# VincentStimper/normalizing-flows

Hardware: AMD Instinct MI355X
Metric: samples/sec + NLL (nats/dim), 32-layer RQ-NSF d=64 B=65536 (higher is better)
Workload: dtype f32; 1 GPU; BASELINE configs[1]: log_prob of 32 x [CoupledRQS(d=64, 2 blocks, 128 hidden, K=8, tail 3) + LULinearPermute(64)] + DiagGaussian, batch 65536 rows/GPU, N(0,I) inputs, sigma=0.01 perturbed seeded weights; rows_per_gpu=65536, global_rows=65536, layers=32, launch=hipGraph replay, parallelism=dp1

## Files before the change

include/nf_mi355x.h:

```cpp
#ifndef NF_MI355X_H
#define NF_MI355X_H

#include <stdint.h>

#ifdef __cplusplus
extern "C" {
#endif

typedef void *nf_stream_t;

enum { NF_OK = 0, NF_EIO = -5, NF_EFAULT = -14, NF_EINVAL = -22, NF_ERANGE = -34, NF_ENOTSUP = -95 };
enum { NF_F32 = 0, NF_F64 = 1 };
enum { NF_LD_WRITE = 0, NF_LD_ADD = 1, NF_LD_SUB = -1 };
enum { NF_TAILS_NONE = 0, NF_TAILS_LINEAR = 1, NF_TAILS_CIRCULAR = 2, NF_TAILS_FEATURE = 3  };
enum { NF_SCALE_EXP = 0, NF_SCALE_SIGMOID = 1, NF_SCALE_SIGMOID_INV = 2, NF_SCALE_NONE = 3 };
enum { NF_RQS_DENSITY = 0, NF_RQS_SAMPLE_IDENTITY = 1, NF_RQS_SAMPLE_TRANSFORM = 2 };

const char *nf_version(void);
const char *nf_strerror(int code);
int nf_mfma_clock_probe(void *out2_u64, void *sink_f32, int iters, nf_stream_t stream);
int nf_max_bins(void);
int nf_persistent_workgroups(void);

int nf_rqs_spline(const void *x, const void *w, int64_t ldw, const void *h, int64_t ldh, const void *d,
// ... 41 lines not shown
                                void *grad_ud, int dtype, const int32_t *tails_t, const void *bound_t,
                                const int32_t *tails_i, const void *bound_i, nf_stream_t stream);

int nf_rqs_fused_final_row(int K, int g, int rb, int rho);
#define NF_RQS_COMPACT_DIFF (1 << 16)
int nf_rqs_fused_compact_row(int K, int rb, int rho);
int64_t nf_rqs_fused_pack_size(int nI, int nT, int hidden, int num_blocks, int K);
int nf_rqs_fused_pack(void *wpack, const void *w_init, const void *b_init, const void *const *w_blocks,
                      const void *const *b_blocks, const void *w_final, const void *b_final, const void *uw,
                      const void *uh, const void *ud, int nI, int nT, int hidden, int num_blocks, int K,
                      double tail_bound, double min_bin_width, double min_bin_height, double min_derivative,
                      nf_stream_t stream);
int nf_rqs_fused_pack_lu(void *wpack, int num_blocks, const int64_t *perm, const void *lower_entries,
                         const void *upper_entries, const void *unconstrained_upper_diag, const void *bias, int D,
                         double eps, int K, nf_stream_t stream);
int nf_rqs_fused(const void *x, void *y, void *logdet, const void *wpack, int mask_parity, int fuse_lu, int64_t B,
                 int D, int hidden, int num_blocks, int K, double tail_bound, double min_bin_width,
                 double min_bin_height, double min_derivative, int direction, int acc, nf_stream_t stream);
int nf_rqs_fused_chain(const void *x, void *y, void *logdet, const void *const *wpacks, const int *mask_parities,
                       int num_layers, int fuse_lu, int64_t B, int D, int hidden, int num_blocks, int K,
                       double tail_bound, double min_bin_width, double min_bin_height, double min_derivative,
                       int direction, int acc, nf_stream_t stream);
int nf_rqs_fused_small_batch(int enable);

int nf_rqs_fused_pack_final(void *wpack, const void *w_final, const void *b_final, const void *uw, const void *uh,
                            const void *ud, int hidden, int num_blocks, int K, double tail_bound, double min_bin_width,
                            double min_bin_height, double min_derivative, nf_stream_t stream);
int nf_rqs_fused_train_fwd(const void *x, const void *h2, void *y, void *logdet, void *cond_out, const void *wpack,
                           int mask_parity, int64_t B, int D, int hidden, int num_blocks, int K, double tail_bound,
                           double min_bin_width, double min_bin_height, double min_derivative, int acc, nf_stream_t stream);
int nf_rqs_fused_pack_all(void *wpack, const void *w_init, const void *b_init, const void *const *w_blocks,
                          const void *const *b_blocks, const void *w_final, const void *b_final, const void *uw, const void *uh,
                          const void *ud, int hidden, int num_blocks, int K, double tail_bound, double min_bin_width,
                          double min_bin_height, double min_derivative, void *wfull, void *wpad, const void *identity_idx,
                          nf_stream_t stream);
int nf_rqs_fused_train_full_fwd(const void *x, void *y, void *logdet, void *cond_out, void *act_out, const void *wpack,
                                int mask_parity, int64_t B, int D, int hidden, int num_blocks, int K, double tail_bound,
                                double min_bin_width, double min_bin_height, double min_derivative, int acc, nf_stream_t stream);
int nf_rqs_fused_pack_all_multi(const void *table, int n_layers, int hidden, int num_blocks, int K, double tail_bound,
                                double min_bin_width, double min_bin_height, double min_derivative, nf_stream_t stream);
int nf_rqs_coupling_bwd_p24(const void *x, const void *grad_y, const void *grad_logdet, const void *cond24, const void *uw,
                            const void *uh, const void *ud, const int64_t *identity_idx, int nI, const int64_t *transform_idx,
                            int nT, int64_t B, int D, double tail_bound, double min_bin_width, double min_bin_height,
                            double min_derivative, double wh_div, void *grad_x, void *grad_cond24, void *grad_uw,
                            void *grad_uh, void *grad_ud, nf_stream_t stream);

// ... 322 lines not shown
```

normalizing-flows_amd/config.py:

```python
fused_gemm = "f32"


def set_fused_gemm(mode):
    global fused_gemm
    if mode not in ("f32", "bf16x3"):
        raise ValueError("fused_gemm must be 'f32' or 'bf16x3'")
    fused_gemm = mode


glow_level_chains = True


def set_glow_level_chains(mode=True):
    global glow_level_chains
    glow_level_chains = bool(mode)


def set_roctx(mode=True):
    from . import _prof
    _prof.enabled = bool(mode)


wgrad_pair = True

# ... 111 lines not shown
    global train_prepack
    train_prepack = bool(mode)


maf_halves = True


def set_maf_halves(mode=True):
    global maf_halves
    maf_halves = bool(mode)


maf_tri = True


def set_maf_tri(mode=True):
    global maf_tri
    maf_tri = bool(mode)


def set_fused_chain(mode=True):
    global fused_chain
    fused_chain = bool(mode)


lu_matvec2 = True


def set_lu_matvec2(mode=True):
    global lu_matvec2
    lu_matvec2 = bool(mode)


made_fused = True


def set_made_fused(mode=True):
    global made_fused
    made_fused = bool(mode)


made_train = True


def set_made_train(mode=True):
    global made_train
# ... 175 lines not shown
```

normalizing-flows_amd/core.py:

```python
import torch
from . import _keys
from . import config as _config
from torch import nn

from . import _prepack
from .flows.base import run_flow
from .flows.mixing import LULinearPermute
from .flows.neural_spline import CoupledRationalQuadraticSpline


def invalidate_caches(module):
    for m in module.modules():
        for k in list(m.__dict__.keys()):
            if k.endswith("_cache") and not k.startswith("__"):
                v = m.__dict__[k]
                m.__dict__[k] = {} if isinstance(v, dict) else None
        if hasattr(m, "refresh_graphs"):
            m.refresh_graphs()
    _realnvp_cache.clear()


def _pair_signature(crqs):
    p = crqs.prqct
    return (p.features, p.transform_net.hidden_features, len(p.transform_net.blocks), p.num_bins, p.tail_bound,
# ... 323 lines not shown
        for o in obj:
            _cached_tensors(o, out, depth + 1)
    elif isinstance(obj, dict) and depth < 4:
        for o in obj.values():
            _cached_tensors(o, out, depth + 1)


def _packed_blobs(owner):
    out = []
    if owner is not None:
        for m in owner.modules():
            for k, v in m.__dict__.items():
                if k.endswith("_cache"):
                    _cached_tensors(v, out)
    _cached_tensors(list(_realnvp_cache.values()), out)
    return out


class _GraphCache:

    def __init__(self, owner=None):
        self.enabled = False
        self.graphs = {}
        self.stamp, self.sig = _keys.stamp(), None
        self.owner = None if owner is None else __import__("weakref").ref(owner)

    def clear(self):
        self.graphs = {}

    def run(self, key, fn, *inputs):
        if not self.enabled:
            return fn(*inputs)
        if self.sig is None or self.stamp != _keys.stamp():
            owner = self.owner() if self.owner is not None else None
            sig = _keys.signature(owner.parameters()) if owner is not None else _keys.stamp()
            if self.sig is not None and sig != self.sig:
                self.graphs = {}
            self.sig, self.stamp = sig, _keys.stamp()
        entry = self.graphs.get(key)
        if entry is None:
            static_in = [t.clone() for t in inputs]
            _config._graph_recording += 1
            try:
                s = torch.cuda.Stream()
                s.wait_stream(torch.cuda.current_stream())
                with torch.cuda.stream(s):
                    fn(*static_in)
                torch.cuda.current_stream().wait_stream(s)
                g = torch.cuda.CUDAGraph()
                with torch.cuda.graph(g):
                    static_out = fn(*static_in)
            finally:
                _config._graph_recording -= 1
            entry = (g, static_in, static_out, _packed_blobs(self.owner() if self.owner is not None else None))
            self.graphs[key] = entry
        g, static_in, static_out = entry[:3]
        for dst, src in zip(static_in, inputs):
            dst.copy_(src)
        g.replay()
        if torch.is_tensor(static_out):
            return static_out.clone()
# ... 43 lines not shown
    def inverse(self, x):
        for i in range(len(self.flows) - 1, -1, -1):
            x, _ = self.flows[i].inverse(x)
        return x

    def inverse_and_log_det(self, x):
        log_det = torch.zeros(len(x), dtype=x.dtype, device=x.device)
        x = run_chain(self.flows, x, True, log_det, +1)
        return x, log_det

    def _train_pad_rows(self, x):
        B = x.shape[0] if x.dim() == 2 else 0
        if (B < 1024 or B % 64 == 0 or not _config.train_pad_batch or not x.is_cuda or x.dtype != torch.float32 or x.shape[1] != 64
                or not torch.is_grad_enabled() or not (_config.train_pair and _config.train_bwd_onecall)):
            return 0
        fl = list(self.flows)
        for a, b in zip(fl[:-1], fl[1:]):
            if (isinstance(a, CoupledRationalQuadraticSpline) and isinstance(b, LULinearPermute) and b.linear.features == 64
                    and a.prqct._train_full_ok(x, None, False) and all(p.requires_grad for p in a.parameters())
                    and all(p.requires_grad for p in b.parameters())):
                return (-B) % 64 if all(_row_wise(f) for f in fl) else 0
        return 0

    def _log_prob_impl(self, x):
        pad = self._train_pad_rows(x)
        if pad:
            B = x.shape[0]
            x = torch.cat([x, x.new_zeros((pad, x.shape[1]))])
        log_q = torch.zeros(len(x), dtype=x.dtype, device=x.device)
        z = run_chain(self.flows, x, True, log_q, +1)
        if hasattr(self.q0, "_log_prob_acc"):
            self.q0._log_prob_acc(z, log_q, +1)
        else:
            log_q += self.q0.log_prob(z)
        return log_q[:B] if pad else log_q

    def log_prob(self, x):
        if self._graphs.enabled and torch.is_grad_enabled() and any(p.requires_grad for p in self.parameters()):
            return self._log_prob_impl(x)
        return self._graphs.run(("log_prob", tuple(x.shape), x.dtype), self._log_prob_impl, x)

    def forward_kld(self, x):
        return -torch.mean(self.log_prob(x))

    def _sample_impl(self, eps):
        z, log_q = self.q0.from_noise(eps)
        z = run_chain(self.flows, z, False, log_q, -1)
        return z, log_q

    def sample_from_noise(self, eps):
        if self._graphs.enabled and torch.is_grad_enabled() and any(p.requires_grad for p in self.parameters()):
            return self._sample_impl(eps)
        return self._graphs.run(("sample", tuple(eps.shape), eps.dtype), self._sample_impl, eps)

    def sample(self, num_samples=1):
        if hasattr(self.q0, "from_noise"):
            eps = torch.randn((num_samples,) + tuple(self.q0.shape), dtype=self.q0.loc.dtype,
                              device=self.q0.loc.device)
            return self.sample_from_noise(eps)
        z, log_q = self.q0(num_samples)
        for flow in self.flows:
            z = run_flow(flow, z, False, log_q, -1)
# ... 319 lines not shown
```

normalizing-flows_amd/csrc/affine.hip:

```cpp
#include "common.hpp"

namespace nf {

template <typename T>
__global__ void __launch_bounds__(256)
masked_affine_kernel(const T *__restrict__ z, const T *__restrict__ b, const T *__restrict__ s,
                     const T *__restrict__ t, T *__restrict__ y, T *__restrict__ logdet, int64_t B, int64_t inner,
                     int direction, int acc) {
    __shared__ T sred[16];
    if constexpr (sizeof(T) == 4) {
        if (inner <= 256 && (inner & 3) == 0) {
            typedef float v4 __attribute__((ext_vector_type(4)));
            const int L4 = (int)inner >> 2;
            int P = 1;
            while (P < L4) P <<= 1;
            const int rpw = 64 / P, lane = threadIdx.x & 63, rin = lane / P, i = lane - rin * P;
            const int64_t wave = ((int64_t)blockIdx.x * blockDim.x + threadIdx.x) >> 6;
            const int64_t nwaves = ((int64_t)gridDim.x * blockDim.x) >> 6;
            const bool col_on = i < L4;
            v4 bi = {0.0f, 0.0f, 0.0f, 0.0f};
            if (col_on) bi = *reinterpret_cast<const v4 *>(reinterpret_cast<const float *>(b) + 4 * i);
            for (int64_t r0 = wave * rpw; r0 < B; r0 += nwaves * rpw) {
                const int64_t r = r0 + rin;
                const bool on = r < B && col_on;
// ... 213 lines not shown
                    for (int e = 0; e < 4; ++e) {
                        const float q = (zv[e] - mu[e]) * inv[e];
                        a += 0.5f * q * q;
                    }
                }
                for (int off = P >> 1; off >= 1; off >>= 1) a += __shfl_xor(a, off, 64);
                if (r < B && i == 0) ld_store(reinterpret_cast<float *>(out) + r, (float)cst - a, acc);
            }
            return;
        }
    }
    for (int64_t r = wave; r < B; r += nwaves) {
        T a = T(0);
        for (int64_t j = lane; j < d; j += 64) {
            const T ls = log_scale[j] + ls_shift;
            const T q = (z[r * d + j] - loc[j]) / M<T>::exp(ls);
            a += ls + T(0.5) * q * q;
        }
        a = wave_sum(a);
        if (lane == 0) ld_store(out + r, cst - a, acc);
    }
}

template <typename T>
__global__ void __launch_bounds__(256)
squeeze_kernel(const T *__restrict__ z, T *__restrict__ y, int64_t B, int C, int H, int W, int direction) {
    const int64_t N = B * (int64_t)C * H * W;
    for (int64_t i = (int64_t)blockIdx.x * blockDim.x + threadIdx.x; i < N; i += (int64_t)gridDim.x * blockDim.x) {
        if (direction == 0) {
            const int Co = C / 4, Ho = 2 * H, Wo = 2 * W;
            int64_t r = i;
            const int wo = (int)(r % Wo); r /= Wo;
            const int ho = (int)(r % Ho); r /= Ho;
            const int co = (int)(r % Co); r /= Co;
            const int ci = 4 * co + 2 * (ho & 1) + (wo & 1);
            y[i] = z[((r * C + ci) * H + (ho >> 1)) * W + (wo >> 1)];
        } else {
            const int Co = 4 * C, Ho = H / 2, Wo = W / 2;
            int64_t r = i;
            const int wo = (int)(r % Wo); r /= Wo;
            const int ho = (int)(r % Ho); r /= Ho;
            const int co = (int)(r % Co); r /= Co;
            const int ci = co >> 2, di = (co >> 1) & 1, dj = co & 1;
            y[i] = z[((r * C + ci) * H + (2 * ho + di)) * W + (2 * wo + dj)];
        }
    }
// ... 127 lines not shown
}

extern "C" int nf_diag_gaussian_log_prob(const void *z, const void *loc, const void *log_scale, double log_scale_shift,
                                         void *out, int64_t B, int64_t d, int acc, int dtype, nf_stream_t stream) {
    if (B < 0 || d < 1 || acc < NF_LD_SUB || acc > NF_LD_ADD) return NF_EINVAL;
    if (B == 0) return NF_OK;
    if (!z || !loc || !log_scale || !out) return NF_EFAULT;
    if (dtype == NF_F32 && d <= 256 && (d & 3) == 0 && nf_misaligned16(z, loc, log_scale)) return NF_EINVAL;
    hipStream_t st = (hipStream_t)stream;
    const double cst = -0.5 * (double)d * log(2.0 * M_PI);
    int grid = grid_for(B, 4);
    if (dtype == NF_F32 && d <= 256 && (d & 3) == 0) grid = grid_for(B * d / 4, 256);
    NF_DISPATCH(dtype,
                hipLaunchKernelGGL(diag_gaussian_kernel<float>, dim3(grid), dim3(256), 0, st, (const float *)z,
                                   (const float *)loc, (const float *)log_scale, (float)log_scale_shift, (float *)out,
                                   B, d, (float)cst, acc),
                hipLaunchKernelGGL(diag_gaussian_kernel<double>, dim3(grid), dim3(256), 0, st, (const double *)z,
                                   (const double *)loc, (const double *)log_scale, log_scale_shift, (double *)out, B,
                                   d, cst, acc));
    NF_CHECK_LAUNCH();
    return NF_OK;
}

extern "C" int nf_squeeze(const void *z, void *y, int64_t B, int C, int H, int W, int direction, int dtype,
                          nf_stream_t stream) {
    if (B < 0 || C < 1 || H < 1 || W < 1 || (direction != 0 && direction != 1)) return NF_EINVAL;
    if (direction == 0 && (C % 4)) return NF_EINVAL;
    if (direction == 1 && ((H % 2) || (W % 2))) return NF_EINVAL;
    if (B == 0) return NF_OK;
    if (!z || !y) return NF_EFAULT;
    hipStream_t st = (hipStream_t)stream;
    const int grid = grid_for(B * (int64_t)C * H * W, 256 * 4);
    NF_DISPATCH(dtype,
                hipLaunchKernelGGL(squeeze_kernel<float>, dim3(grid), dim3(256), 0, st, (const float *)z, (float *)y, B,
                                   C, H, W, direction),
                hipLaunchKernelGGL(squeeze_kernel<double>, dim3(grid), dim3(256), 0, st, (const double *)z,
                                   (double *)y, B, C, H, W, direction));
    NF_CHECK_LAUNCH();
    return NF_OK;
}

extern "C" int nf_maf_affine(const void *x, const void *params, void *y, void *logdet, int64_t B, int D, int direction,
                             int acc, int dtype, nf_stream_t stream) {
    if (B < 0 || D < 1 || (direction != 0 && direction != 1) || acc < NF_LD_SUB || acc > NF_LD_ADD) return NF_EINVAL;
    if (B == 0) return NF_OK;
    if (!x || !params || !y) return NF_EFAULT;
// ... 11 lines not shown
```

normalizing-flows_amd/csrc/common.hpp:

```cpp
#pragma once
#include <hip/hip_runtime.h>
#include <stdint.h>
#include <math.h>

#include "../../include/nf_mi355x.h"

#define NF_MAX_BINS 64
#define NF_WAVE 64

#ifdef NF_SAFE_WAITS
#define NF_WAIT_VMCNT(N) asm volatile("s_waitcnt vmcnt(0)" ::: "memory")
#else
#define NF_WAIT_VMCNT(N) asm volatile("s_waitcnt vmcnt(%0)" ::"n"(N) : "memory")
#endif

#define NF_DMA16(BASE, BYTE_OFF, LDS_DST)                                                                                          \
    do {                                                                                                                           \
        uint32_t m0__;                                                                                                             \
        const uint32_t ldsa__ = __builtin_amdgcn_readfirstlane((uint32_t)(uintptr_t)(LDS_DST));                                    \
        const uint64_t b64__ = (uint64_t)(uintptr_t)(BASE);                                                                        \
        const uint64_t sb__ = ((uint64_t)(uint32_t)__builtin_amdgcn_readfirstlane((uint32_t)(b64__ >> 32)) << 32) |                \
                              (uint32_t)__builtin_amdgcn_readfirstlane((uint32_t)b64__);                                           \
        asm volatile("s_mov_b32 %0, m0\n\ts_mov_b32 m0, %1\n\ts_nop 0\n\tglobal_load_lds_dwordx4 %2, %3\n\ts_mov_b32 m0, %0"      \
                     : "=&s"(m0__) : "s"(ldsa__), "v"((uint32_t)(BYTE_OFF)), "s"(sb__) : "memory");                                \
// ... 288 lines not shown
template <typename T> __device__ __forceinline__ T wave_sum(T v) {
#pragma unroll
    for (int o = 32; o > 0; o >>= 1) v += __shfl_xor(v, o, 64);
    return v;
}

template <typename T> __device__ __forceinline__ T block_sum(T v, T *scratch ) {
    v = wave_sum(v);
    const int lane = threadIdx.x & 63, wid = threadIdx.x >> 6, nw = (blockDim.x + 63) >> 6;
    __syncthreads();
    if (lane == 0) scratch[wid] = v;
    __syncthreads();
    T r = T(0);
    for (int i = 0; i < nw; ++i) r += scratch[i];
    return r;
}

template <typename T> __device__ __forceinline__ void ld_store(T *dst, T v, int acc) {
    if (acc == NF_LD_WRITE) *dst = v;
    else if (acc == NF_LD_ADD) *dst += v;
    else *dst -= v;
}

static inline int grid_for(int64_t work_items, int per_block, int max_blocks = 256 * 8) {
    int64_t g = (work_items + per_block - 1) / per_block;
    if (g < 1) g = 1;
    if (g > max_blocks) g = max_blocks;
    return (int)g;
}

constexpr int NF_PERSISTENT_WORKGROUPS = 256;
static inline int persistent_grid(int64_t ntiles) {
    return (int)(ntiles < NF_PERSISTENT_WORKGROUPS ? ntiles : NF_PERSISTENT_WORKGROUPS);
}

constexpr int NF_MAX_DEVICES = 64;
struct LdsOptIn {
    size_t opted[NF_MAX_DEVICES];
};
inline int opt_in_lds(const void *kernel, size_t lds, LdsOptIn &state) {
    if (lds <= 64 * 1024) return NF_OK;
    int dev = 0;
    if (hipGetDevice(&dev) != hipSuccess || dev < 0 || dev >= NF_MAX_DEVICES) return NF_EIO;
    if (lds <= state.opted[dev]) return NF_OK;
    if (hipFuncSetAttribute(kernel, hipFuncAttributeMaxDynamicSharedMemorySize, (int)lds) != hipSuccess) return NF_ENOTSUP;
    state.opted[dev] = lds;
// ... 5 lines not shown
```

normalizing-flows_amd/csrc/rqs_fused.hip:

```cpp
#include "fused_common.hpp"
#include <type_traits>

#define NF_TRAIN_STORE(ptr, val) __builtin_nontemporal_store((val), (ptr))

#ifdef NF_FUSED_SECONDARY
#define rqs_fused_kernel rqs_fused_kernel_nw4
#endif

namespace nf {

#ifndef NF_FUSED_SECONDARY
__global__ void pack_init_kernel(const float *__restrict__ W , const float *__restrict__ b, float *__restrict__ stage,
                                 float *__restrict__ bias_dst) {
    for (int i = blockIdx.x * blockDim.x + threadIdx.x; i < F_STAGE; i += gridDim.x * blockDim.x) {
        const int r4 = i & 3, lane = (i >> 2) & 63, s = (i >> 8) & 3, m = i >> 10;
        const int row = 32 * m + (lane & 31);
        const int k = 8 * s + 4 * (lane >> 5) + r4;
        stage[i] = W[row * F_NI + k];
    }
    for (int i = blockIdx.x * blockDim.x + threadIdx.x; i < 128; i += gridDim.x * blockDim.x) {
        const int reg = i & 15, hh = (i >> 4) & 1, m = i >> 5;
        bias_dst[i] = b[32 * m + 8 * (reg >> 2) + 4 * hh + (reg & 3)];
    }
}
// ... 288 lines not shown
    }
}

#ifndef NF_FUSED_WAVES
#define NF_FUSED_WAVES 8
#endif
constexpr int F_NW = NF_FUSED_WAVES;
constexpr int F_DMA_WAVES = 4 < F_NW ? 4 : F_NW;
constexpr int F_THREADS = 64 * F_NW;
constexpr int F_ROWS = 32 * F_NW;

struct FlowArgs {
    const float *blob[F_MAX_LAYERS];
    unsigned long long parity;
    int nlayers;
    int ngroups;
};

template <int DIR, bool LU, int TRAIN = 0, int KB = F_K, int HB = 4>
__global__ void __launch_bounds__(F_THREADS, 2)
rqs_fused_kernel(const float *__restrict__ x, float *__restrict__ y, float *__restrict__ logdet, FlowArgs fa,
                 int64_t B, int nblk, RqsParams<float> p, int acc, const float *__restrict__ h_in = nullptr,
                 float *__restrict__ cond_out = nullptr, float unscale = 1.0f, float *__restrict__ act_out = nullptr,
                 float *__restrict__ xlu_out = nullptr) {
    extern __shared__ __attribute__((aligned(16))) float smem[];
    constexpr int LA = (HB == 4 && !(DIR == 0 && LU) && TRAIN == 0) ? 1 : 2;
    static_assert(KB == 4 || KB == 8 || KB == 16, "bins");
    static_assert(!TRAIN || (KB == F_K && DIR == 0 && (!LU || TRAIN == 2)),
                  "the training variants: 8 bins, density direction; the fused LU only with the whole-layer forward (TRAIN = 2)");
    static_assert(HB == 4 || ((HB == 2 || HB == 1) && !TRAIN), "hidden row-blocks");
    constexpr bool COMPACT = KB == 8 && TRAIN == 0;
    constexpr bool RAW_RELU = !(KB == 16 && DIR == 0 && LU && HB == 4);
    auto relu_acc = [](float v) __attribute__((always_inline)) { return RAW_RELU ? relu_raw(v) : fmaxf(v, 0.0f); };
    constexpr bool PAIR_TAB = TRAIN == 0;
    constexpr int MP = 3 * KB, FPL = 16 / KB, GQ = KB / 4, TABW = 3 * (KB + 1);
    FusedLayout lay;
    lay.nblk = nblk;
    lay.K = KB;
    float *ring = smem;
    float *stash = ring + 2 * F_STAGE;
    float *small2 = stash + F_NW * 32 * 64;
    const int small_pitch = TRAIN ? lay.small_padded_legacy() : lay.small_padded();
    const int tid = threadIdx.x, lane = tid & 63, hh = lane >> 5;
    const int wid = __builtin_amdgcn_readfirstlane(tid >> 6);
    const int64_t row = (int64_t)blockIdx.x * F_ROWS + wid * 32 + (lane & 31);
    const bool valid = row < B;
    const int nhid = 2 * nblk * HB;
// ... 413 lines not shown
#pragma unroll
            for (int f = 0; f < FPL; ++f) element(g, f);
        }
        if (DIR == 0) uncond_group(g);
    }

    if (LU && DIR == 1) {
        float yin[32];
#pragma unroll
        for (int c = 0; c < 32; ++c) yin[c] = st[c * 64];
        const float *bsrc = small + lay.off_bias_lu(1) + hh * 16;
        f32x16 o0 = load_bias16(bsrc), o1 = load_bias16(bsrc + 32);
        lu_mm(acquire(), lane, yin, o0, o1);
#pragma unroll
        for (int c = 0; c < 16; ++c) {
            st[c * 64] = o0[c];
            st[(16 + c) * 64] = o1[c];
        }
        if (hh == 0) ld -= lu_lad;
    }
    }

    ld += __shfl_xor(ld, 32, 64);
    if (valid) {
#pragma unroll
        for (int Q = 0; Q < 4; ++Q) {
            f32x4 a, b;
#pragma unroll
            for (int c = 0; c < 4; ++c) {
                a[c] = st[(8 * Q + c) * 64];
                b[c] = st[(8 * Q + 4 + c) * 64];
            }
            float *dst = y + row * F_D + 16 * Q + 8 * hh;
            *reinterpret_cast<f32x4 *>(dst) = a;
            *reinterpret_cast<f32x4 *>(dst + 4) = b;
        }
        if (hh == 0) ld_store(logdet + row, ld, acc);
    }
}

#ifndef NF_FUSED_SECONDARY
struct PackAllArgs {
    const float *w_init, *b_init, *w_final, *b_final, *uw, *uh, *ud;
    const float *w_blk[32], *b_blk[32];
    int nblk;
    float *wfull, *wpad;
    const int64_t *iidx;
};
__device__ __forceinline__ void pack_all_body(const PackAllArgs &a, float *__restrict__ blob, float wh_scale,
                                              const RqsParams<float> &p) {
    FusedLayout lay;
    lay.nblk = a.nblk;
    float *small = blob + F_HDR, *stages = blob + lay.off_stages();
    const int nlin = 2 * a.nblk, nst = 1 + 4 * nlin + 24;
    const int64_t tid0 = (int64_t)blockIdx.x * blockDim.x + threadIdx.x, nth = (int64_t)gridDim.x * blockDim.x;
    for (int64_t i = tid0; i < (int64_t)nst * F_STAGE; i += nth) {
        const int st = (int)(i >> 12), j = (int)(i & (F_STAGE - 1));
        const int r4 = j & 3, lane = (j >> 2) & 63;
// ... 321 lines not shown
    if (!wpack || !perm || !lower_entries || !upper_entries || !unconstrained_upper_diag || !bias) return NF_EFAULT;
    hipStream_t st = (hipStream_t)stream;
    FusedLayout lay;
    lay.nblk = num_blocks;
    lay.K = K;
    float *blob = (float *)wpack;
    float *small = blob + F_HDR;
    float *stages = blob + lay.off_stages();
    const size_t lds = (size_t)4 * F_D * F_D * sizeof(double) + F_D * sizeof(int) + F_D * sizeof(double) + 64;
    static LdsOptIn opted = {};
    if (opt_in_lds(reinterpret_cast<const void *>(&pack_lu_kernel), lds, opted) != NF_OK) return NF_ENOTSUP;
    hipLaunchKernelGGL(pack_lu_kernel, dim3(1), dim3(256), lds, st, perm, (const float *)lower_entries,
                       (const float *)upper_entries, (const float *)unconstrained_upper_diag, (const float *)bias,
                       (float)eps, stages + (size_t)lay.lu_stage(0) * F_STAGE, stages + (size_t)lay.lu_stage(1) * F_STAGE,
                       small + lay.off_bias_lu(0), small + lay.off_bias_lu(1), blob);
    NF_CHECK_LAUNCH();
    return NF_OK;
}

#endif

template <int DIR, bool LU, int KB, int HB>
static int launch_fused(const void *x, void *y, void *logdet, const FlowArgs &fa, int64_t B, int num_blocks,
                        const RqsParams<float> &p, int acc, size_t lds, hipStream_t st) {
    static LdsOptIn opted = {};
    if (opt_in_lds(reinterpret_cast<const void *>(&rqs_fused_kernel<DIR, LU, false, KB, HB>), lds, opted) != NF_OK) return NF_ENOTSUP;
    const int grid = (int)((B + F_ROWS - 1) / F_ROWS);
    hipLaunchKernelGGL((rqs_fused_kernel<DIR, LU, false, KB, HB>), dim3(grid), dim3(F_THREADS), lds, st, (const float *)x, (float *)y,
                       (float *)logdet, fa, B, num_blocks, p, acc, (const float *)nullptr, (float *)nullptr, 1.0f);
    NF_CHECK_LAUNCH();
    return NF_OK;
}

static int chain_dispatch(const void *x, void *y, void *logdet, const FlowArgs &fa, int64_t B, int hidden, int num_blocks, int K,
                          const RqsParams<float> &p, int direction, int fuse_lu, int acc, hipStream_t st) {
    FusedLayout lay;
    lay.nblk = num_blocks;
    lay.K = K;
    const size_t lds = (size_t)(2 * F_STAGE + F_NW * 32 * 64 + 2 * lay.small_padded()) * sizeof(float);
    if (lds > 160 * 1024) return NF_ENOTSUP;
#define NF_FUSED_DISPATCH(KB, HB)                                                                                     \
    do {                                                                                                              \
        if (direction == 0)                                                                                           \
            return fuse_lu ? launch_fused<0, true, KB, HB>(x, y, logdet, fa, B, num_blocks, p, acc, lds, st)          \
                           : launch_fused<0, false, KB, HB>(x, y, logdet, fa, B, num_blocks, p, acc, lds, st);        \
        return fuse_lu ? launch_fused<1, true, KB, HB>(x, y, logdet, fa, B, num_blocks, p, acc, lds, st)              \
                       : launch_fused<1, false, KB, HB>(x, y, logdet, fa, B, num_blocks, p, acc, lds, st);            \
    } while (0)
    if (hidden == F_H / 2) {
        if (K == 4) NF_FUSED_DISPATCH(4, 2);
        if (K == 16) NF_FUSED_DISPATCH(16, 2);
        NF_FUSED_DISPATCH(8, 2);
    }
    if (hidden == F_H / 4) {
        if (K == 4) NF_FUSED_DISPATCH(4, 1);
        if (K == 16) NF_FUSED_DISPATCH(16, 1);
        NF_FUSED_DISPATCH(8, 1);
    }
    if (K == 4) NF_FUSED_DISPATCH(4, 4);
    if (K == 16) NF_FUSED_DISPATCH(16, 4);
    NF_FUSED_DISPATCH(8, 4);
#undef NF_FUSED_DISPATCH
}

#ifdef NF_FUSED_SECONDARY
extern "C" int nf_rqs_fused_chain_nw4_(const void *x, void *y, void *logdet, const void *fa, int64_t B, int hidden, int num_blocks, int K,
                                       const void *p, int direction, int fuse_lu, int acc, nf_stream_t stream) {
    static_assert(F_NW == 4, "the secondary build is the 4-wave one");
    return chain_dispatch(x, y, logdet, *static_cast<const FlowArgs *>(fa), B, hidden, num_blocks, K,
                          *static_cast<const RqsParams<float> *>(p), direction, fuse_lu, acc, (hipStream_t)stream);
}
#else
extern "C" int nf_rqs_fused_chain_nw4_(const void *x, void *y, void *logdet, const void *fa, int64_t B, int hidden, int num_blocks, int K,
                                       const void *p, int direction, int fuse_lu, int acc, nf_stream_t stream);

extern "C" int nf_rqs_fused_small_batch(int enable) {
    const int old = g_small_batch;
    if (enable >= 0) g_small_batch = enable ? 1 : 0;
    return old;
}

extern "C" int nf_rqs_fused_chain(const void *x, void *y, void *logdet, const void *const *wpacks,
                                  const int *mask_parities, int num_layers, int fuse_lu, int64_t B, int D, int hidden,
                                  int num_blocks, int K, double tail_bound, double min_bin_width, double min_bin_height,
                                  double min_derivative, int direction, int acc, nf_stream_t stream) {
    if ((D != F_D && D != 16 && D != 32 && D != 48) || (hidden != F_H && hidden != F_H / 2 && hidden != F_H / 4) || !fused_bins_ok(K) ||
        num_blocks < 0 || num_blocks > 16)
        return NF_ENOTSUP;
    if (num_layers < 1 || num_layers > F_MAX_LAYERS) return NF_ERANGE;
    if (min_bin_width * K > 1.0 || min_bin_height * K > 1.0) return NF_EINVAL;
    if (B < 0 || (direction != 0 && direction != 1)) return NF_EINVAL;
    if (acc < NF_LD_SUB || acc > NF_LD_ADD) return NF_EINVAL;
    if (B == 0) return NF_OK;
    if (!x || !y || !logdet || !wpacks || !mask_parities) return NF_EFAULT;
    if (nf_misaligned16(x, y)) return NF_EINVAL;
    FlowArgs fa;
    fa.parity = 0ull;
    fa.nlayers = num_layers;
    fa.ngroups = (D / 16) * (K / 4);
    for (int l = 0; l < F_MAX_LAYERS; ++l) fa.blob[l] = nullptr;
    for (int l = 0; l < num_layers; ++l) {
        if (!wpacks[l]) return NF_EFAULT;
        if (mask_parities[l] != 0 && mask_parities[l] != 1) return NF_EINVAL;
        if (nf_misaligned16(wpacks[l])) return NF_EINVAL;
        fa.blob[l] = (const float *)wpacks[l];
        if (mask_parities[l]) fa.parity |= 1ull << l;
    }
    auto p = make_rqs_params<float>(K, NF_TAILS_LINEAR, tail_bound, 0, 1, 0, 1, min_bin_width, min_bin_height,
                                    min_derivative, sqrt((double)F_H));
    if (g_small_batch && B <= NF_FUSED_SMALL_ROWS)
        return nf_rqs_fused_chain_nw4_(x, y, logdet, &fa, B, hidden, num_blocks, K, &p, direction, fuse_lu, acc, stream);
    return chain_dispatch(x, y, logdet, fa, B, hidden, num_blocks, K, p, direction, fuse_lu, acc, (hipStream_t)stream);
}

extern "C" int nf_rqs_fused_train_fwd(const void *x, const void *h2, void *y, void *logdet, void *cond_out, const void *wpack,
                                      int mask_parity, int64_t B, int D, int hidden, int num_blocks, int K, double tail_bound,
                                      double min_bin_width, double min_bin_height, double min_derivative, int acc,
                                      nf_stream_t stream) {
    if (D != F_D || hidden != F_H || K != F_K || num_blocks < 0 || num_blocks > 16) return NF_ENOTSUP;
    if (B < 0 || (mask_parity != 0 && mask_parity != 1) || acc < NF_LD_SUB || acc > NF_LD_ADD) return NF_EINVAL;
    if (B == 0) return NF_OK;
    if (!x || !h2 || !y || !logdet || !cond_out || !wpack) return NF_EFAULT;
    if (nf_misaligned16(x, h2, y, cond_out, wpack)) return NF_EINVAL;
    FlowArgs fa;
    fa.parity = mask_parity ? 1ull : 0ull;
    fa.nlayers = 1;
    fa.ngroups = F_K;
    for (int l = 0; l < F_MAX_LAYERS; ++l) fa.blob[l] = nullptr;
    fa.blob[0] = (const float *)wpack;
    FusedLayout lay;
    lay.nblk = num_blocks;
    auto p = make_rqs_params<float>(K, NF_TAILS_LINEAR, tail_bound, 0, 1, 0, 1, min_bin_width, min_bin_height,
                                    min_derivative, sqrt((double)hidden));
    const size_t lds = (size_t)(2 * F_STAGE + F_NW * 32 * 64 + lay.small_padded_legacy() + F_NW * 1536) * sizeof(float);
    if (lds > 160 * 1024) return NF_ENOTSUP;
// ... 21 lines not shown
```

normalizing-flows_amd/distributions.py:

```python
import numpy as np
import torch
from . import _keys
from torch import nn

from . import ops
from .autograd import DiagGaussianLogProbFn, GaussianRowsLogProbFn, needs_grad


class BaseDistribution(nn.Module):
    def __init__(self):
        super().__init__()

    def forward(self, num_samples=1):
        raise NotImplementedError

    def log_prob(self, z):
        raise NotImplementedError

    def sample(self, num_samples=1, **kwargs):
        z, _ = self.forward(num_samples, **kwargs)
        return z


class DiagGaussian(BaseDistribution):
# ... 31 lines not shown
            return z, log_p
        log_scale = self.log_scale.detach() + self._shift()
        z = self.loc.detach() + torch.exp(log_scale) * eps
        zeros = torch.zeros_like(self.loc.detach())
        log_p = ops.diag_gaussian_log_prob(eps, zeros, zeros, 0.0)
        log_p = log_p - log_scale.sum()
        return z, log_p

    def log_prob(self, z, context=None):
        if needs_grad(z, self.loc, self.log_scale):
            return DiagGaussianLogProbFn.apply(z, self.loc, self.log_scale, self._shift())
        return ops.diag_gaussian_log_prob(z, self.loc.detach(), self.log_scale.detach(), self._shift())

    def _log_prob_acc(self, z, log_q, acc=+1):
        if needs_grad(z, self.loc, self.log_scale):
            lp = self.log_prob(z)
            if acc > 0:
                log_q += lp
            else:
                log_q -= lp
            return log_q
        ops.diag_gaussian_log_prob(z, self.loc.detach(), self.log_scale.detach(), self._shift(), out=log_q, acc=acc)
        return log_q


class UniformGaussian(BaseDistribution):

    def __init__(self, ndim, ind, scale=None):
        super().__init__()
        self.ndim = ndim
        if isinstance(ind, int):
            ind = [ind]
        if torch.is_tensor(ind):
            self.register_buffer("ind", ind.long())
        else:
            self.register_buffer("ind", torch.tensor(ind, dtype=torch.long))
        uniform = set(self.ind.tolist())
        self.register_buffer("ind_", torch.tensor([i for i in range(self.ndim) if i not in uniform], dtype=torch.long))
        perm_ = torch.cat((self.ind, self.ind_))
        inv_perm_ = torch.zeros_like(perm_)
        inv_perm_[perm_] = torch.arange(self.ndim)
        self.register_buffer("inv_perm", inv_perm_)
        self.register_buffer("scale", torch.ones(self.ndim) if scale is None else scale)

    def forward(self, num_samples=1, context=None):
        z = self.sample(num_samples)
# ... 203 lines not shown
```

normalizing-flows_amd/ops.py:

```python
import ctypes as C
import math

import torch

from . import _lib as L
from ._lib import ptr, ptr_any


def _ld_buffer(logdet, acc, B, like, want=True):
    if logdet is None and want:
        return torch.empty(B, dtype=like.dtype, device=like.device), L.LD_WRITE
    return logdet, L.LD_ADD if acc is None else acc


def _a16(t, vec=True):
    if t is None or not vec or t.data_ptr() % 16 == 0:
        return t
    return torch.empty(t.shape, dtype=t.dtype, device=t.device).copy_(t)


def _ld_acc(logdet, acc):
    return (L.LD_ADD if logdet is not None and acc is None else acc) or 0


# ... 891 lines not shown
    x = x.contiguous()
    params = params.contiguous()
    B, D = x.shape
    gx = torch.empty_like(x)
    gparams = torch.empty_like(params)
    gy = None if gy is None else gy.contiguous()
    gld = None if gld is None else gld.contiguous()
    L.call("nf_maf_affine_bwd", ptr(x), ptr(params), ptr(gy), ptr(gld), ptr(gx), ptr(gparams), B, D, direction, L.dtype_code(x),
           L.stream())
    return gx, gparams


def maf_implicit_sweep(x, params, gx, gld, gxm, v, gp, changed):
    L.require_device(x, params, gx, gld, gxm, v, gp, changed)
    B, D = x.shape
    L.call("nf_maf_implicit_sweep", ptr(x), ptr(params), ptr(gx), ptr(gld), ptr(gxm), ptr(v), ptr(gp), ptr(changed), B, D,
           L.dtype_code(x), L.stream())


def rqs_fused_chain(x, blobs, parities, hidden, num_blocks, K, direction, logdet=None, acc=None, tail_bound=3.0,
                    min_bin_width=1e-3, min_bin_height=1e-3, min_derivative=1e-3, fuse_lu=True, live_d=None):
    return _rqs_fused_launch("nf_rqs_fused_chain", x, blobs, parities, hidden, num_blocks, K, direction, logdet,
                             acc, (tail_bound, min_bin_width, min_bin_height, min_derivative), fuse_lu, live_d, padded_rows=True)


def rqs_fused_x3_chain(x, blobs, parities, hidden, num_blocks, K, direction, logdet=None, acc=None, tail_bound=3.0,
                       min_bin_width=1e-3, min_bin_height=1e-3, min_derivative=1e-3, fuse_lu=True, live_d=None):
    return _rqs_fused_launch("nf_rqs_fused_x3_chain", x, blobs, parities, hidden, num_blocks, K, direction,
                             logdet, acc, (tail_bound, min_bin_width, min_bin_height, min_derivative), fuse_lu)


def nsf_wide_tables(uw, uh, ud, K, tail_bound, min_bin_width=1e-3, min_bin_height=1e-3, min_derivative=1e-3):
    L.require_device(uw, uh, ud, dtype=torch.float32)
    tabs = torch.empty(uw.shape[0], 3 * (K + 1), dtype=torch.float32, device=uw.device)
    L.call("nf_nsf_wide_tables", ptr(uw.contiguous()), ptr(uh.contiguous()), ptr(ud.contiguous()), ptr(tabs), uw.shape[0], K,
           float(tail_bound), min_bin_width, min_bin_height, min_derivative, L.stream())
    return tabs


def nsf_wide(x, blob, table, tabs, hidden_padded, direction, tail_bound, min_bin_width=1e-3, min_bin_height=1e-3,
             min_derivative=1e-3, logdet=None, acc=None, lu_logdet=None, K=8):
    L.require_device(x, blob, table, tabs, lu_logdet, dtype=torch.float32)
    if x.dtype != torch.float32:
        raise NotImplementedError("nsf_wide: float32 only")
    B, D = x.shape
    x = _a16(x.contiguous(), D % 4 == 0)
# ... 735 lines not shown
```

Before: 13.11 million samples/s.

## Fuse DiagGaussian base log-prob into fused RQS chain kernel epilogue

Adds a precomputed base-distribution block (inverse scales, loc, log-scale sums, constant) and folds the DiagGaussian log-density into the epilogue of the fused coupling chain kernel. The final latent z is then never written to global memory, and the separate base log-prob kernel launch goes away. The Python route args are also cached per shape so graph replay bypasses the generic graph path. The cost is a narrower fast path (d=64, f32, specific layer pairing) and a small change in the summation order of the log-prob.

Result: no change. 13.18 million samples/s, median of 6 (+0.5%).

```diff
diff --git a/include/nf_mi355x.h b/include/nf_mi355x.h
--- a/include/nf_mi355x.h
+++ b/include/nf_mi355x.h
@@ -87,6 +87,13 @@
                        double tail_bound, double min_bin_width, double min_bin_height, double min_derivative,
                        int direction, int acc, nf_stream_t stream);
 int nf_rqs_fused_small_batch(int enable);
+int64_t nf_diag_gaussian_base_block_floats(int64_t d);
+int nf_diag_gaussian_base_block(const void *loc, const void *log_scale, double log_scale_shift, void *block, int64_t d, int dtype,
+                                nf_stream_t stream);
+int nf_rqs_fused_chain_base(const void *x, void *y, void *log_prob, const void *base_block, const void *const *wpacks,
+                            const int *mask_parities, int num_layers, int fuse_lu, int64_t B, int D, int hidden, int num_blocks,
+                            int K, double tail_bound, double min_bin_width, double min_bin_height, double min_derivative,
+                            nf_stream_t stream);
 
 int nf_rqs_fused_pack_final(void *wpack, const void *w_final, const void *b_final, const void *uw, const void *uh,
                             const void *ud, int hidden, int num_blocks, int K, double tail_bound, double min_bin_width,
diff --git a/normalizing-flows_amd/config.py b/normalizing-flows_amd/config.py
--- a/normalizing-flows_amd/config.py
+++ b/normalizing-flows_amd/config.py
@@ -157,6 +157,14 @@
 def set_fused_chain(mode=True):
     global fused_chain
     fused_chain = bool(mode)
+
+
+chain_base = True
+
+
+def set_chain_base(mode=True):
+    global chain_base
+    chain_base = bool(mode)
 
 
 lu_matvec2 = True
diff --git a/normalizing-flows_amd/core.py b/normalizing-flows_amd/core.py
--- a/normalizing-flows_amd/core.py
+++ b/normalizing-flows_amd/core.py
@@ -369,21 +369,26 @@
     def __init__(self, owner=None):
         self.enabled = False
         self.graphs = {}
+        self.direct = {}
         self.stamp, self.sig = _keys.stamp(), None
         self.owner = None if owner is None else __import__("weakref").ref(owner)
 
     def clear(self):
         self.graphs = {}
-
-    def run(self, key, fn, *inputs):
-        if not self.enabled:
-            return fn(*inputs)
+        self.direct = {}
+
+    def validate(self):
         if self.sig is None or self.stamp != _keys.stamp():
             owner = self.owner() if self.owner is not None else None
             sig = _keys.signature(owner.parameters()) if owner is not None else _keys.stamp()
             if self.sig is not None and sig != self.sig:
-                self.graphs = {}
+                self.clear()
             self.sig, self.stamp = sig, _keys.stamp()
+
+    def run(self, key, fn, *inputs):
+        if not self.enabled:
+            return fn(*inputs)
+        self.validate()
         entry = self.graphs.get(key)
         if entry is None:
             static_in = [t.clone() for t in inputs]
@@ -473,7 +478,47 @@
                 return (-B) % 64 if all(_row_wise(f) for f in fl) else 0
         return 0
 
+    def _chain_base_route(self, x):
+        fl = list(self.flows)
+        n = len(fl)
+        if not (_config.chain_base and _config.fused_chain and _config.fused_gemm == "f32" and torch.is_tensor(x) and x.dim() == 2
+                and x.shape[0] > 0 and x.shape[1] == 64 and x.dtype == torch.float32 and x.is_cuda and n % 2 == 0 and 4 <= n <= 128
+                and hasattr(self.q0, "_base_block")):
+            return None
+        pairs = [(fl[i], fl[i + 1]) for i in range(n - 2, -1, -2)]
+        if not all(isinstance(a, CoupledRationalQuadraticSpline) and isinstance(b, LULinearPermute) for a, b in pairs):
+            return None
+        p0 = pairs[0][0].prqct
+        if not all(a.prqct.features == 64 and a.prqct.use_fused and a._pair_eligible(x, b) and a.prqct._fused_eligible(x, None)
+                   and _pair_signature(a) == _pair_signature(pairs[0][0]) for a, b in pairs):
+            return None
+        block = self.q0._base_block()
+        if block is None:
+            return None
+        feats, hidden, nblk, K, tb, mw, mh, md = _pair_signature(pairs[0][0])
+        return (block, [a.prqct._fused_blob(b) for a, b in pairs], [a.prqct._fused_parity for a, b in pairs], p0._fused_hidden(), nblk, K,
+                tb, mw, mh, md)
+
+    def _chain_base_args(self, x):
+        g = self._graphs
+        if not g.enabled:
+            return self._chain_base_route(x)
+        key = ("log_prob", tuple(x.shape), x.dtype, x.device, _config.chain_base, _config.fused_chain, _config.fused_gemm,
+               torch.is_grad_enabled() and x.requires_grad)
+        g.validate()
+        if key not in g.direct:
+            g.direct[key] = self._chain_base_route(x)
+        return g.direct[key]
+
+    def _log_prob_chain_base(self, x, args):
+        from . import _prof, ops
+        with _prof.range_("rqs_fused_chain_base[%d x (CoupledRQS + LULinearPermute) + DiagGaussian]" % len(args[1])):
+            return ops.rqs_fused_chain_base(x, *args, fuse_lu=True)
+
     def _log_prob_impl(self, x):
+        args = self._chain_base_args(x)
+        if args is not None:
+            return self._log_prob_chain_base(x, args)
         pad = self._train_pad_rows(x)
         if pad:
             B = x.shape[0]
@@ -489,6 +534,10 @@
     def log_prob(self, x):
         if self._graphs.enabled and torch.is_grad_enabled() and any(p.requires_grad for p in self.parameters()):
             return self._log_prob_impl(x)
+        if self._graphs.enabled:
+            args = self._chain_base_args(x)
+            if args is not None:
+                return self._log_prob_chain_base(x, args)
         return self._graphs.run(("log_prob", tuple(x.shape), x.dtype), self._log_prob_impl, x)
 
     def forward_kld(self, x):
diff --git a/normalizing-flows_amd/csrc/affine.hip b/normalizing-flows_amd/csrc/affine.hip
--- a/normalizing-flows_amd/csrc/affine.hip
+++ b/normalizing-flows_amd/csrc/affine.hip
@@ -259,6 +259,29 @@
     }
 }
 
+__global__ void __launch_bounds__(64)
+diag_gaussian_base_block_kernel(const float *__restrict__ loc, const float *__restrict__ log_scale, float ls_shift, float cst,
+                                float *__restrict__ block) {
+    typedef float v4 __attribute__((ext_vector_type(4)));
+    const int i = threadIdx.x;
+    if (i < NF_BASE_D / 4) {
+        const v4 mu = *reinterpret_cast<const v4 *>(loc + 4 * i);
+        const v4 lsv = *reinterpret_cast<const v4 *>(log_scale + 4 * i);
+        v4 inv;
+        float lsum = 0.0f;
+#pragma unroll
+        for (int e = 0; e < 4; ++e) {
+            const float ls = lsv[e] + ls_shift;
+            inv[e] = 1.0f / M<float>::exp(ls);
+            lsum += ls;
+        }
+        *reinterpret_cast<v4 *>(block + NF_BASE_INV + 4 * i) = inv;
+        *reinterpret_cast<v4 *>(block + NF_BASE_LOC + 4 * i) = mu;
+        block[NF_BASE_LSUM + i] = lsum;
+        block[NF_BASE_CST + i] = i == 0 ? cst : 0.0f;
+    }
+}
+
 template <typename T>
 __global__ void __launch_bounds__(256)
 squeeze_kernel(const T *__restrict__ z, T *__restrict__ y, int64_t B, int C, int H, int W, int direction) {
@@ -432,6 +455,20 @@
     return NF_OK;
 }
 
+extern "C" int64_t nf_diag_gaussian_base_block_floats(int64_t d) { return d == NF_BASE_D ? NF_BASE_FLOATS : NF_ENOTSUP; }
+
+extern "C" int nf_diag_gaussian_base_block(const void *loc, const void *log_scale, double log_scale_shift, void *block, int64_t d,
+                                           int dtype, nf_stream_t stream) {
+    if (d != NF_BASE_D || dtype != NF_F32) return NF_ENOTSUP;
+    if (!loc || !log_scale || !block) return NF_EFAULT;
+    if (nf_misaligned16(loc, log_scale, block)) return NF_EINVAL;
+    const double cst = -0.5 * (double)d * log(2.0 * M_PI);
+    hipLaunchKernelGGL(diag_gaussian_base_block_kernel, dim3(1), dim3(64), 0, (hipStream_t)stream, (const float *)loc,
+                       (const float *)log_scale, (float)log_scale_shift, (float)cst, (float *)block);
+    NF_CHECK_LAUNCH();
+    return NF_OK;
+}
+
 extern "C" int nf_squeeze(const void *z, void *y, int64_t B, int C, int H, int W, int direction, int dtype,
                           nf_stream_t stream) {
     if (B < 0 || C < 1 || H < 1 || W < 1 || (direction != 0 && direction != 1)) return NF_EINVAL;
diff --git a/normalizing-flows_amd/csrc/common.hpp b/normalizing-flows_amd/csrc/common.hpp
--- a/normalizing-flows_amd/csrc/common.hpp
+++ b/normalizing-flows_amd/csrc/common.hpp
@@ -334,6 +334,24 @@
     else *dst -= v;
 }
 
+constexpr int NF_BASE_D = 64;
+constexpr int NF_BASE_INV = 0, NF_BASE_LOC = 64, NF_BASE_LSUM = 128, NF_BASE_CST = 144, NF_BASE_FLOATS = 160;
+
+template <typename V4>
+__device__ __forceinline__ float base_group(float lsum, const V4 &z, const V4 &loc, const V4 &inv) {
+#pragma clang fp contract(off)
+    float a = lsum;
+#pragma unroll
+    for (int e = 0; e < 4; ++e) {
+        const float d = z[e] - loc[e];
+        const float q = d * inv[e];
+        const float h = q * 0.5f;
+        const float u = q * h;
+        a = a + u;
+    }
+    return a;
+}
+
 static inline int grid_for(int64_t work_items, int per_block, int max_blocks = 256 * 8) {
     int64_t g = (work_items + per_block - 1) / per_block;
     if (g < 1) g = 1;
diff --git a/normalizing-flows_amd/csrc/rqs_fused.hip b/normalizing-flows_amd/csrc/rqs_fused.hip
--- a/normalizing-flows_amd/csrc/rqs_fused.hip
+++ b/normalizing-flows_amd/csrc/rqs_fused.hip
@@ -334,7 +334,7 @@
 rqs_fused_kernel(const float *__restrict__ x, float *__restrict__ y, float *__restrict__ logdet, FlowArgs fa,
                  int64_t B, int nblk, RqsParams<float> p, int acc, const float *__restrict__ h_in = nullptr,
                  float *__restrict__ cond_out = nullptr, float unscale = 1.0f, float *__restrict__ act_out = nullptr,
-                 float *__restrict__ xlu_out = nullptr) {
+                 float *__restrict__ xlu_out = nullptr, const float *__restrict__ base = nullptr) {
     extern __shared__ __attribute__((aligned(16))) float smem[];
     constexpr int LA = (HB == 4 && !(DIR == 0 && LU) && TRAIN == 0) ? 1 : 2;
     static_assert(KB == 4 || KB == 8 || KB == 16, "bins");
@@ -794,18 +794,45 @@
     }
 
     ld += __shfl_xor(ld, 32, 64);
+    bool store_rows = true;
+    if constexpr (DIR == 0 && TRAIN == 0) {
+        if (base) {
+            float aj[4][2];
+#pragma unroll
+            for (int Q = 0; Q < 4; ++Q) {
+                const float *bq = base + 16 * Q + 8 * hh;
+#pragma unroll
+                for (int j = 0; j < 2; ++j) {
+                    const f32x4 inv = *reinterpret_cast<const f32x4 *>(bq + NF_BASE_INV + 4 * j);
+                    const f32x4 mu = *reinterpret_cast<const f32x4 *>(bq + NF_BASE_LOC + 4 * j);
+                    f32x4 zv;
+#pragma unroll
+                    for (int e = 0; e < 4; ++e) zv[e] = st[(8 * Q + 4 * j + e) * 64];
+                    aj[Q][j] = base_group(base[NF_BASE_LSUM + 4 * Q + 2 * hh + j], zv, mu, inv);
+                }
+            }
+            float t0 = (aj[0][0] + aj[2][0]) + (aj[1][0] + aj[3][0]);
+            float t1 = (aj[0][1] + aj[2][1]) + (aj[1][1] + aj[3][1]);
+            t0 += __shfl_xor(t0, 32, 64);
+            t1 += __shfl_xor(t1, 32, 64);
+            ld = (base[NF_BASE_CST] - (t0 + t1)) + ld;
+            store_rows = y != nullptr;
+        }
+    }
     if (valid) {
-#pragma unroll
-        for (int Q = 0; Q < 4; ++Q) {
-            f32x4 a, b;
-#pragma unroll
-            for (int c = 0; c < 4; ++c) {
-                a[c] = st[(8 * Q + c) * 64];
-                b[c] = st[(8 * Q + 4 + c) * 64];
-            }
-            float *dst = y + row * F_D + 16 * Q + 8 * hh;
-            *reinterpret_cast<f32x4 *>(dst) = a;
-            *reinterpret_cast<f32x4 *>(dst + 4) = b;
+        if (store_rows) {
+#pragma unroll
+            for (int Q = 0; Q < 4; ++Q) {
+                f32x4 a, b;
+#pragma unroll
+                for (int c = 0; c < 4; ++c) {
+                    a[c] = st[(8 * Q + c) * 64];
+                    b[c] = st[(8 * Q + 4 + c) * 64];
+                }
+                float *dst = y + row * F_D + 16 * Q + 8 * hh;
+                *reinterpret_cast<f32x4 *>(dst) = a;
+                *reinterpret_cast<f32x4 *>(dst + 4) = b;
+            }
         }
         if (hh == 0) ld_store(logdet + row, ld, acc);
     }
@@ -1173,18 +1200,19 @@
 
 template <int DIR, bool LU, int KB, int HB>
 static int launch_fused(const void *x, void *y, void *logdet, const FlowArgs &fa, int64_t B, int num_blocks,
-                        const RqsParams<float> &p, int acc, size_t lds, hipStream_t st) {
+                        const RqsParams<float> &p, int acc, size_t lds, hipStream_t st, const float *base) {
     static LdsOptIn opted = {};
     if (opt_in_lds(reinterpret_cast<const void *>(&rqs_fused_kernel<DIR, LU, false, KB, HB>), lds, opted) != NF_OK) return NF_ENOTSUP;
     const int grid = (int)((B + F_ROWS - 1) / F_ROWS);
     hipLaunchKernelGGL((rqs_fused_kernel<DIR, LU, false, KB, HB>), dim3(grid), dim3(F_THREADS), lds, st, (const float *)x, (float *)y,
-                       (float *)logdet, fa, B, num_blocks, p, acc, (const float *)nullptr, (float *)nullptr, 1.0f);
+                       (float *)logdet, fa, B, num_blocks, p, acc, (const float *)nullptr, (float *)nullptr, 1.0f, (float *)nullptr,
+                       (float *)nullptr, base);
     NF_CHECK_LAUNCH();
     return NF_OK;
 }
 
 static int chain_dispatch(const void *x, void *y, void *logdet, const FlowArgs &fa, int64_t B, int hidden, int num_blocks, int K,
-                          const RqsParams<float> &p, int direction, int fuse_lu, int acc, hipStream_t st) {
+                          const RqsParams<float> &p, int direction, int fuse_lu, int acc, hipStream_t st, const float *base) {
     FusedLayout lay;
     lay.nblk = num_blocks;
     lay.K = K;
@@ -1193,10 +1221,10 @@
 #define NF_FUSED_DISPATCH(KB, HB)                                                                                     \
     do {                                                                                                              \
         if (direction == 0)                                                                                           \
-            return fuse_lu ? launch_fused<0, true, KB, HB>(x, y, logdet, fa, B, num_blocks, p, acc, lds, st)          \
-                           : launch_fused<0, false, KB, HB>(x, y, logdet, fa, B, num_blocks, p, acc, lds, st);        \
-        return fuse_lu ? launch_fused<1, true, KB, HB>(x, y, logdet, fa, B, num_blocks, p, acc, lds, st)              \
-                       : launch_fused<1, false, KB, HB>(x, y, logdet, fa, B, num_blocks, p, acc, lds, st);            \
+            return fuse_lu ? launch_fused<0, true, KB, HB>(x, y, logdet, fa, B, num_blocks, p, acc, lds, st, base)    \
+                           : launch_fused<0, false, KB, HB>(x, y, logdet, fa, B, num_blocks, p, acc, lds, st, base);  \
+        return fuse_lu ? launch_fused<1, true, KB, HB>(x, y, logdet, fa, B, num_blocks, p, acc, lds, st, base)        \
+                       : launch_fused<1, false, KB, HB>(x, y, logdet, fa, B, num_blocks, p, acc, lds, st, base);      \
     } while (0)
     if (hidden == F_H / 2) {
         if (K == 4) NF_FUSED_DISPATCH(4, 2);
@@ -1216,14 +1244,14 @@
 
 #ifdef NF_FUSED_SECONDARY
 extern "C" int nf_rqs_fused_chain_nw4_(const void *x, void *y, void *logdet, const void *fa, int64_t B, int hidden, int num_blocks, int K,
-                                       const void *p, int direction, int fuse_lu, int acc, nf_stream_t stream) {
+                                       const void *p, int direction, int fuse_lu, int acc, nf_stream_t stream, const void *base) {
     static_assert(F_NW == 4, "the secondary build is the 4-wave one");
     return chain_dispatch(x, y, logdet, *static_cast<const FlowArgs *>(fa), B, hidden, num_blocks, K,
-                          *static_cast<const RqsParams<float> *>(p), direction, fuse_lu, acc, (hipStream_t)stream);
+                          *static_cast<const RqsParams<float> *>(p), direction, fuse_lu, acc, (hipStream_t)stream, (const float *)base);
 }
 #else
 extern "C" int nf_rqs_fused_chain_nw4_(const void *x, void *y, void *logdet, const void *fa, int64_t B, int hidden, int num_blocks, int K,
-                                       const void *p, int direction, int fuse_lu, int acc, nf_stream_t stream);
+                                       const void *p, int direction, int fuse_lu, int acc, nf_stream_t stream, const void *base);
 
 extern "C" int nf_rqs_fused_small_batch(int enable) {
     const int old = g_small_batch;
@@ -1231,10 +1259,9 @@
     return old;
 }
 
-extern "C" int nf_rqs_fused_chain(const void *x, void *y, void *logdet, const void *const *wpacks,
-                                  const int *mask_parities, int num_layers, int fuse_lu, int64_t B, int D, int hidden,
-                                  int num_blocks, int K, double tail_bound, double min_bin_width, double min_bin_height,
-                                  double min_derivative, int direction, int acc, nf_stream_t stream) {
+static int chain_entry(const void *x, void *y, void *logdet, const void *const *wpacks, const int *mask_parities, int num_layers,
+                       int fuse_lu, int64_t B, int D, int hidden, int num_blocks, int K, double tail_bound, double min_bin_width,
+                       double min_bin_height, double min_derivative, int direction, int acc, nf_stream_t stream, const void *base) {
     if ((D != F_D && D != 16 && D != 32 && D != 48) || (hidden != F_H && hidden != F_H / 2 && hidden != F_H / 4) || !fused_bins_ok(K) ||
         num_blocks < 0 || num_blocks > 16)
         return NF_ENOTSUP;
@@ -1243,8 +1270,8 @@
     if (B < 0 || (direction != 0 && direction != 1)) return NF_EINVAL;
     if (acc < NF_LD_SUB || acc > NF_LD_ADD) return NF_EINVAL;
     if (B == 0) return NF_OK;
-    if (!x || !y || !logdet || !wpacks || !mask_parities) return NF_EFAULT;
-    if (nf_misaligned16(x, y)) return NF_EINVAL;
+    if (!x || (!y && !base) || !logdet || !wpacks || !mask_parities) return NF_EFAULT;
+    if (nf_misaligned16(x, y, base)) return NF_EINVAL;
     FlowArgs fa;
     fa.parity = 0ull;
     fa.nlayers = num_layers;
@@ -1260,8 +1287,27 @@
     auto p = make_rqs_params<float>(K, NF_TAILS_LINEAR, tail_bound, 0, 1, 0, 1, min_bin_width, min_bin_height,
                                     min_derivative, sqrt((double)F_H));
     if (g_small_batch && B <= NF_FUSED_SMALL_ROWS)
-        return nf_rqs_fused_chain_nw4_(x, y, logdet, &fa, B, hidden, num_blocks, K, &p, direction, fuse_lu, acc, stream);
-    return chain_dispatch(x, y, logdet, fa, B, hidden, num_blocks, K, p, direction, fuse_lu, acc, (hipStream_t)stream);
+        return nf_rqs_fused_chain_nw4_(x, y, logdet, &fa, B, hidden, num_blocks, K, &p, direction, fuse_lu, acc, stream, base);
+    return chain_dispatch(x, y, logdet, fa, B, hidden, num_blocks, K, p, direction, fuse_lu, acc, (hipStream_t)stream,
+                          (const float *)base);
+}
+
+extern "C" int nf_rqs_fused_chain(const void *x, void *y, void *logdet, const void *const *wpacks,
+                                  const int *mask_parities, int num_layers, int fuse_lu, int64_t B, int D, int hidden,
+                                  int num_blocks, int K, double tail_bound, double min_bin_width, double min_bin_height,
+                                  double min_derivative, int direction, int acc, nf_stream_t stream) {
+    return chain_entry(x, y, logdet, wpacks, mask_parities, num_layers, fuse_lu, B, D, hidden, num_blocks, K, tail_bound, min_bin_width,
+                       min_bin_height, min_derivative, direction, acc, stream, nullptr);
+}
+
+extern "C" int nf_rqs_fused_chain_base(const void *x, void *y, void *log_prob, const void *base_block, const void *const *wpacks,
+                                       const int *mask_parities, int num_layers, int fuse_lu, int64_t B, int D, int hidden,
+                                       int num_blocks, int K, double tail_bound, double min_bin_width, double min_bin_height,
+                                       double min_derivative, nf_stream_t stream) {
+    if (D != F_D) return NF_ENOTSUP;
+    if (B > 0 && !base_block) return NF_EFAULT;
+    return chain_entry(x, y, log_prob, wpacks, mask_parities, num_layers, fuse_lu, B, D, hidden, num_blocks, K, tail_bound,
+                       min_bin_width, min_bin_height, min_derivative, 0, NF_LD_WRITE, stream, base_block);
 }
 
 extern "C" int nf_rqs_fused_train_fwd(const void *x, const void *h2, void *y, void *logdet, void *cond_out, const void *wpack,
diff --git a/normalizing-flows_amd/distributions.py b/normalizing-flows_amd/distributions.py
--- a/normalizing-flows_amd/distributions.py
+++ b/normalizing-flows_amd/distributions.py
@@ -77,6 +77,14 @@
             return log_q
         ops.diag_gaussian_log_prob(z, self.loc.detach(), self.log_scale.detach(), self._shift(), out=log_q, acc=acc)
         return log_q
+
+    def _base_block(self):
+        if (type(self) is not DiagGaussian or self.shape != (64,) or self.loc.dtype != torch.float32 or not self.loc.is_cuda
+                or self.log_scale.dtype != torch.float32 or needs_grad(self.loc, self.log_scale)):
+            return None
+        shift = self._shift()
+        return _keys.pcached(self, "_base_block_cache", [self.loc, self.log_scale], (shift,),
+                             lambda: ops.diag_gaussian_base_block(self.loc.detach(), self.log_scale.detach(), shift))
 
 
 class UniformGaussian(BaseDistribution):
diff --git a/normalizing-flows_amd/ops.py b/normalizing-flows_amd/ops.py
--- a/normalizing-flows_amd/ops.py
+++ b/normalizing-flows_amd/ops.py
@@ -937,6 +937,31 @@
                     min_bin_width=1e-3, min_bin_height=1e-3, min_derivative=1e-3, fuse_lu=True, live_d=None):
     return _rqs_fused_launch("nf_rqs_fused_chain", x, blobs, parities, hidden, num_blocks, K, direction, logdet,
                              acc, (tail_bound, min_bin_width, min_bin_height, min_derivative), fuse_lu, live_d, padded_rows=True)
+
+
+def diag_gaussian_base_block(loc, log_scale, log_scale_shift=0.0):
+    L.require_device(loc, log_scale, dtype=torch.float32)
+    d = loc.numel()
+    L.check_count("diag_gaussian_base_block", "log_scale", log_scale, d, "d = %d elements of loc" % d)
+    block = torch.empty(L.size("nf_diag_gaussian_base_block_floats", d), dtype=torch.float32, device=loc.device)
+    L.call("nf_diag_gaussian_base_block", ptr(_a16(loc.contiguous()).view(-1)), ptr(_a16(log_scale.contiguous()).view(-1)),
+           log_scale_shift, ptr(block), d, L.NF_F32, L.stream())
+    return block
+
+
+def rqs_fused_chain_base(x, base_block, blobs, parities, hidden, num_blocks, K, tail_bound=3.0, min_bin_width=1e-3,
+                         min_bin_height=1e-3, min_derivative=1e-3, fuse_lu=True):
+    L.require_device(x, base_block, *blobs, dtype=torch.float32)
+    x = _a16(x.contiguous())
+    B, D = x.shape
+    if D != 64:
+        raise ValueError("nf_rqs_fused_chain_base: rows of 64 live columns")
+    L.check_count("rqs_fused_chain_base", "base_block", base_block, L.size("nf_diag_gaussian_base_block_floats", D), "the base block")
+    log_prob = torch.empty(B, dtype=x.dtype, device=x.device)
+    L.call("nf_rqs_fused_chain_base", ptr(x), ptr(None), ptr(log_prob), ptr(base_block), _ptr_array(blobs),
+           (C.c_int * len(blobs))(*[int(v) for v in parities]), len(blobs), int(fuse_lu), B, D, hidden, num_blocks, K,
+           tail_bound, min_bin_width, min_bin_height, min_derivative, L.stream())
+    return log_prob
 
 
 def rqs_fused_x3_chain(x, blobs, parities, hidden, num_blocks, K, direction, logdet=None, acc=None, tail_bound=3.0,
```
